# angelvillar96/STLPose

Measured on AMD Instinct MI355X. Metric: images/sec/GPU HRNet-W32 384x288 train step; PCKh@0.5 parity, higher is better.
Workload: dtype f16/bf16; 1 GPU; HRNet-W32 384x288 bs=32/GPU train step (fwd+MSE+bwd+Adam), random-init weights; global_batch=32, parallelism=dp1

## Files before the change

### include/stlpose_hip.h

```cpp
#ifndef STLPOSE_HIP_H
#define STLPOSE_HIP_H
#include <stdint.h>
#ifdef __cplusplus
extern "C" {
#endif

#define STL_F32 0
#define STL_BF16 1
#define STL_F16 2
#define STL_NSHARD 2

#define STL_DT2(grad_dtype, fwd_dtype) ((grad_dtype) | ((fwd_dtype) << 8))

#define STL_SRC_PLAIN 0
#define STL_SRC_BN 1
#define STL_SRC_BNBWD 2
#define STL_SRC_BNADD 3

typedef struct stl_src {
    const void* x;
    const void* y;
    int32_t mode;
    int32_t relu;
    const double* stats;
// ... 127 lines not shown
typedef struct stl_bnrec {
    int64_t stats_off;
    int64_t param_off;
    int64_t buf_off;
    int32_t C;
    float inv_count;
} stl_bnrec;
int stl_bn_running_update(const double* stats, float* buffers, int64_t* num_batches_tracked ,
                          const stl_bnrec* tab, int n, float momentum, int32_t* overflow, void* stream);
int stl_bn_param_grads(const double* rstats, float* grads, const stl_bnrec* tab, int n, void* stream);

int stl_adam_step(float* p, const float* g, float* m, float* v, int64_t n, const float* hyper,
                  int32_t* step, const int32_t* overflow , void* stream);
int stl_sgd_step(float* p, const float* g, float* mom, int64_t n, const float* hyper, int32_t* step,
                 const int32_t* overflow , void* stream);

int stl_affine_crop(const uint8_t* src, const int64_t* src_off, const int32_t* src_hw, const float* minv, const int32_t* flip,
                    float* out, int B, int Ho, int Wo, const float* mean3, const float* std3, void* stream);
int stl_maxpool2x2(int dtype, const void* x, void* out, int B, int H, int W, int C, void* stream);
int stl_l1_partial(int dtype, const void* a, const void* b, int64_t n, double* partial, int nblk,
                   void* stream);
int stl_l2_partial(int dtype, const void* a, const void* b, int64_t n, double* partial, int nblk, void* stream);
int stl_maxpool2x2_backward(int dtype, const void* x, const void* dy, void* dx, int B, int H, int W, int C, int mask, void* stream);
int stl_l2_backward(int dtype, const void* a, const void* b, void* g, int64_t n, const float* scale, int mask, void* stream);
int stl_bilinear_nchw(const float* in, float* out, int B, int C, int H, int W, int Ho, int Wo,
                      void* stream);
int stl_sum_partials(const double* partial, int n, double scale, float* out, int accumulate, void* stream);

int stl_nchw_to_nhwc(int dtype, const float* in, void* out, int B, int C, int H, int W, void* stream);
int stl_nhwc_to_nchw(int dtype, const void* in, float* out, int B, int C, int H, int W, void* stream);
// ... 143 lines not shown
```

### stlpose_amd/capi.py

```python
from __future__ import annotations

import ctypes as C
import os

_HERE = os.path.dirname(os.path.abspath(__file__))
LIB_PATH = os.environ.get("STLPOSE_HIP_LIB") or os.path.join(_HERE, "libstlpose_hip.so")

F32, BF16, F16 = 0, 1, 2


def dt2(grad_dtype: int, fwd_dtype: int) -> int:
    return grad_dtype | ((fwd_dtype if fwd_dtype != grad_dtype else 0) << 8)


POSE_APPROACH = {"all_kpts": 0, "full_body": 1, "upper_body": 2}
POSE_DIM = {"all_kpts": 34, "full_body": 26, "upper_body": 18}
POSE_METHOD = {"euclidean": 0, "cosine": 1, "manhattan": 2, "confidence": 3, "oks": 4, "l2sq": 5, "cos_normalised": 6}
POSE_PEN = {"zero_coord": 0, "none": 1, "mean": 2, "max": 3}
POSE_TOPK_MAX, POSE_RANK_MAX, POSE_RANK_LABELS_MAX, POSE_NSCORES = 1024, 16384, 4, 10
BOX_MAX, RESIZE_SRC_MAX, RESIZE_DST_MAX = 4096, 16384, 2048
DET_NMS_MAX = 65536
GATHER_COPY, GATHER_UP, GATHER_POOL = 0, 1, 2

MIXED = dt2(BF16, F16)
# ... 36 lines not shown


class FuseBwd(C.Structure):
    _fields_ = [("dtype", i32), ("B", i32), ("H", i32), ("W", i32), ("C", i32), ("ngrads", i32), ("relu", i32),
                ("nbn", i32), ("dz", vp * 4), ("z", vp), ("du", vp), ("bn", Src * 4), ("rstats", vp * 4), ("ydtype", i32), ("pad_", i32)]


class UpBwd(C.Structure):
    _fields_ = [("dtype", i32), ("B", i32), ("H", i32), ("W", i32), ("C", i32), ("shift", i32),
                ("du", vp), ("dt", vp), ("bn", Src), ("rstats", vp), ("ydtype", i32), ("pad_", i32)]


class WPrep(C.Structure):
    _fields_ = [("src_off", i64), ("fwd_off", i64), ("bwd_off", i64), ("Co", i32), ("Ci", i32), ("ks", i32),
                ("Cip", i32), ("patch", i32), ("blk0", i32)]


class Slab(C.Structure):
    _fields_ = [("part_off", i64), ("grad_off", i64), ("nsplit", i32), ("Co", i32), ("Ci", i32), ("ks", i32),
                ("Cip", i32), ("patch", i32), ("blk0", i32), ("pad", i32)]


class BNRec(C.Structure):
    _fields_ = [("stats_off", i64), ("param_off", i64), ("buf_off", i64), ("C", i32), ("inv_count", f32)]


class Patch(C.Structure):
    _fields_ = [("dtype", i32), ("B", i32), ("H", i32), ("W", i32), ("stride", i32), ("pad_", i32), ("img", vp), ("out", vp),
                ("mean3", vp), ("std3", vp)]

# ... 65 lines not shown
    "stl_head_forward": [i32, vp, vp, vp, vp, i32, i32, i32, i32, i32, vp],
    "stl_head_backward": [i32, vp, vp, vp, vp, vp, i32, i32, i32, i32, i32, i32, vp],
    "stl_mse_loss": [vp, vp, vp, vp, vp, i32, vp, i32, i32, i32, f32, vp],
    "stl_gaussian_targets": [vp, vp, vp, vp, i32, i32, i32, i32, f32, f32, f32, vp],
    "stl_heatmap_argmax": [vp, vp, vp, vp, i32, i32, i32, vp],
    "stl_flip_merge": [vp, vp, vp, vp, i32, i32, i32, i32, vp],
    "stl_flip_merge_backward": [vp, vp, vp, vp, i32, i32, i32, i32, vp],
    "stl_final_preds": [vp, vp, vp, vp, vp, i32, i32, i32, i32, vp],
    "stl_weight_prep": [i32, vp, vp, vp, i32, i32, vp],
    "stl_reduce_slabs": [vp, vp, vp, i32, i32, vp],
    "stl_reduce_slabs_range": [C.POINTER(ReduceRange), vp],
    "stl_bn_running_update": [vp, vp, vp, vp, i32, f32, vp, vp],
    "stl_bn_param_grads": [vp, vp, vp, i32, vp],
    "stl_adam_step": [vp, vp, vp, vp, i64, vp, vp, vp, vp],
    "stl_sgd_step": [vp, vp, vp, i64, vp, vp, vp, vp],
    "stl_affine_crop": [vp, vp, vp, vp, vp, vp, i32, i32, i32, vp, vp, vp],
    "stl_maxpool2x2": [i32, vp, vp, i32, i32, i32, i32, vp],
    "stl_l1_partial": [i32, vp, vp, i64, vp, i32, vp],
    "stl_l2_partial": [i32, vp, vp, i64, vp, i32, vp],
    "stl_maxpool2x2_backward": [i32, vp, vp, vp, i32, i32, i32, i32, i32, vp],
    "stl_l2_backward": [i32, vp, vp, vp, i64, vp, i32, vp],
    "stl_bilinear_nchw": [vp, vp, i32, i32, i32, i32, i32, i32, vp],
    "stl_sum_partials": [vp, i32, C.c_double, vp, i32, vp],
    "stl_nchw_to_nhwc": [i32, vp, vp, i32, i32, i32, i32, vp],
    "stl_nhwc_to_nchw": [i32, vp, vp, i32, i32, i32, i32, vp],
    "stl_program_create": [C.POINTER(Op), i32, i32, C.POINTER(vp)],
    "stl_program_run": [vp, C.POINTER(vp)],
    "stl_program_run_range": [vp, C.POINTER(vp), i32, i32],
    "stl_program_destroy": [vp],
    "stl_program_wait_op": [vp, i32, vp],
# ... 65 lines not shown
```

### stlpose_amd/csrc/elementwise.hip

```cpp
#include "common.cuh"

namespace {

template <typename T>
__device__ __forceinline__ void load8(const void* base, size_t elem, float* f) {
    if constexpr (sizeof(T) == 2) {
        unpack<T>(ldg16((const char*)base + elem * 2), f);
    } else {
        unpack<float>(ldg16((const char*)base + elem * 4), f);
        unpack<float>(ldg16((const char*)base + elem * 4 + 16), f + 4);
    }
}
template <typename T>
__device__ __forceinline__ void store8(void* base, size_t elem, const float* f) {
    if constexpr (sizeof(T) == 2) {
        stg16((char*)base + elem * 2, pack<T>(f));
    } else {
        stg16((char*)base + elem * 4, pack<float>(f));
        stg16((char*)base + elem * 4 + 16, pack<float>(f + 4));
    }
}

template <int NS>
__device__ __forceinline__ void flush_sets(float (*acc)[8], float* red, int C, int VPC, double* const* dst,
// ... 636 lines not shown
    uint2 u;
    u.x = (uint32_t)__builtin_bit_cast(unsigned short, v[0]) | ((uint32_t)__builtin_bit_cast(unsigned short, v[1]) << 16);
    u.y = (uint32_t)__builtin_bit_cast(unsigned short, v[2]) | ((uint32_t)__builtin_bit_cast(unsigned short, v[3]) << 16);
    *reinterpret_cast<uint2*>(dst) = u;
}
__device__ __forceinline__ void store_vec4(f16* dst, const f16* v) {
    uint2 u;
    u.x = (uint32_t)__builtin_bit_cast(unsigned short, v[0]) | ((uint32_t)__builtin_bit_cast(unsigned short, v[1]) << 16);
    u.y = (uint32_t)__builtin_bit_cast(unsigned short, v[2]) | ((uint32_t)__builtin_bit_cast(unsigned short, v[3]) << 16);
    *reinterpret_cast<uint2*>(dst) = u;
}
__device__ __forceinline__ void store_vec4(float* dst, const float* v) {
    *reinterpret_cast<float4*>(dst) = make_float4(v[0], v[1], v[2], v[3]);
}

template <typename T, typename TF = T>
__global__ __launch_bounds__(256) void weight_prep_kernel(const float* master, T* wk, const stl_wprep* tab, int n, int blk_base) {
    static_assert(sizeof(T) == sizeof(TF), "both layouts live in one buffer of equal-width elements");
    TF* wkf = reinterpret_cast<TF*>(wk);
    const int bx = blockIdx.x + blk_base;
    const int ei = find_entry(&tab[0].blk0, sizeof(stl_wprep) / 4, n, bx);
    const stl_wprep e = tab[ei];
    const int t = e.ks * e.ks;
    const int64_t tot = (int64_t)e.Co * e.Ci * t;
    const int64_t base = (int64_t)(bx - e.blk0) * 1024;
    if (!e.patch && (e.Ci & 3) == 0 && (e.Co & 3) == 0 && t <= 9 && e.Cip == e.Ci && (e.fwd_off & 3) == 0 && (e.bwd_off < 0 || (e.bwd_off & 3) == 0)) {
        __shared__ float st[32 * (32 * 9 + 1)];
        const int pitch = 32 * t + 1;
        const int tci = (e.Ci + 31) >> 5, ntiles = ((e.Co + 31) >> 5) * tci;
        const int nblk = (int)((tot + 1023) / 1024);
        const float* src0 = master + e.src_off;
        for (int tile = bx - e.blk0; tile < ntiles; tile += nblk) {
            const int co0 = (tile / tci) * 32, ci0 = (tile % tci) * 32;
            const int nco = min(32, e.Co - co0), nci = min(32, e.Ci - ci0), seg = nci * t;
            __syncthreads();
            if (((e.src_off & 3) | (int)((uintptr_t)master & 15)) == 0) {
                const int nv = seg >> 2, ntask = nco * nv;
                float4 buf[9];
#pragma unroll
                for (int u = 0; u < 9; ++u) {
                    const int i = threadIdx.x + u * 256;
                    const bool ok = i < ntask;
                    const int r = ok ? i / nv : 0, q = ok ? i - r * nv : 0;
                    buf[u] = *reinterpret_cast<const float4*>(src0 + ((int64_t)(co0 + r) * e.Ci + ci0) * t + 4 * q);
                }
#pragma unroll
                for (int u = 0; u < 9; ++u) {
                    const int i = threadIdx.x + u * 256;
                    if (i < ntask) {
                        const int r = i / nv, q = i - r * nv;
                        float* d = st + r * pitch + 4 * q;
                        d[0] = buf[u].x, d[1] = buf[u].y, d[2] = buf[u].z, d[3] = buf[u].w;
                    }
                }
            } else {
                for (int r = threadIdx.x >> 6; r < nco; r += 4) {
                    const float* row = src0 + ((int64_t)(co0 + r) * e.Ci + ci0) * t;
                    for (int c = threadIdx.x & 63; c < seg; c += 64) st[r * pitch + c] = row[c];
                }
            }
            __syncthreads();
            T v[4];
            TF vf[4];
            const int q4 = nci >> 2;
            for (int i = threadIdx.x; i < nco * t * q4; i += 256) {
                const int row = q4 == 8 ? i >> 3 : i / q4, c4 = (i - row * q4) * 4;
                const int r = t == 9 ? row / 9 : (t == 1 ? row : row / t), tap = row - r * t;
#pragma unroll
                for (int j = 0; j < 4; ++j) vf[j] = (TF)st[r * pitch + (c4 + j) * t + tap];
                store_vec4(wkf + e.fwd_off + ((int64_t)(co0 + r) * t + tap) * e.Ci + ci0 + c4, vf);
            }
            if (e.bwd_off >= 0) {
                const int p4 = nco >> 2;
                for (int i = threadIdx.x; i < nci * t * p4; i += 256) {
                    const int row = p4 == 8 ? i >> 3 : i / p4, r4 = (i - row * p4) * 4;
                    const int c = t == 9 ? row / 9 : (t == 1 ? row : row / t), tapf = row - c * t;
#pragma unroll
                    for (int j = 0; j < 4; ++j) v[j] = (T)st[(r4 + j) * pitch + c * t + (t - 1 - tapf)];
                    store_vec4(wk + e.bwd_off + ((int64_t)(ci0 + c) * t + tapf) * e.Co + co0 + r4, v);
                }
            }
        }
        return;
    }
    for (int r = 0; r < 4; ++r) {
        const int64_t i = base + r * 256 + threadIdx.x;
        if (i >= tot) return;
        const int co = (int)(i / (e.Ci * t)), rem = (int)(i - (int64_t)co * e.Ci * t), ci = rem / t, tap = rem - ci * t;
        const float v = master[e.src_off + i];
        if (e.patch)
            wkf[e.fwd_off + (int64_t)co * e.Cip + tap * e.Ci + ci] = (TF)v;
        else
            wkf[e.fwd_off + ((int64_t)co * t + tap) * e.Cip + ci] = (TF)v;
        if (e.bwd_off >= 0) {
            if (e.patch)
                wk[e.bwd_off + (int64_t)(tap * e.Ci + ci) * e.Co + co] = (T)v;
            else
                wk[e.bwd_off + ((int64_t)ci * t + (t - 1 - tap)) * e.Co + co] = (T)v;
        }
    }
}

__global__ __launch_bounds__(256) void reduce_slabs_kernel(const float* partials, float* grads, const stl_slab* tab, int n, int blk_base) {
    const int bx = blockIdx.x + blk_base;
    const int ei = find_entry(&tab[0].blk0, sizeof(stl_slab) / 4, n, bx);
    const stl_slab e = tab[ei];
    const int t = e.ks * e.ks;
    const int64_t tot = (int64_t)e.Co * e.Ci * t;
    const int tk = e.patch ? 1 : t, cik = e.patch ? e.Cip : e.Ci;
    const int64_t slab = e.pad ? (int64_t)e.pad : (int64_t)e.Co * tk * cik;
    const int64_t base = (int64_t)(bx - e.blk0) * 1024;
    if (!e.patch && (e.Ci & 3) == 0) {
        const int64_t j = base + 4 * threadIdx.x;
        if (j >= tot) return;
        const float* src = partials + e.part_off + j;
// ... 78 lines not shown
        double r1 = 0.0, r2 = 0.0;
        for (int k = 0; k < STL_NSHARD; ++k) {
            r1 += rstats[e.stats_off + (int64_t)k * 2 * e.C + c];
            r2 += rstats[e.stats_off + (int64_t)k * 2 * e.C + e.C + c];
        }
        grads[e.param_off + c] = (float)r2;
        grads[e.param_off + e.C + c] = (float)r1;
    }
}

__global__ void inc_step_kernel(int32_t* step, const int32_t* overflow) {
    const int t = step[0] < 0 ? -step[0] - 1 : step[0];
    step[0] = (overflow && overflow[0] != 0x7fffffff) ? -t - 1 : t + 1;
}

__global__ __launch_bounds__(256) void adam_kernel(float* p, const float* g, float* m, float* v, int64_t n,
                                                   const float* hyper, const int32_t* step) {
    const float lr = hyper[0], b1 = hyper[1], b2 = hyper[2], eps = hyper[3], wd = hyper[4], gs = hyper[7];
    const int t = step[0];
    if (t < 0) return;
    const float bc1 = 1.f - powf(b1, (float)t), bc2 = 1.f - powf(b2, (float)t);
    const float step_size = lr / bc1, isq2 = 1.f / sqrtf(bc2);
    for (int64_t i = (int64_t)blockIdx.x * 256 + threadIdx.x; i < n; i += (int64_t)gridDim.x * 256) {
        float gi = g[i] * gs;
        if (!(fabsf(gi) <= 3.4e38f)) continue;
        const float pi = p[i];
        if (wd != 0.f) gi = fmaf(wd, pi, gi);
        const float mi = b1 * m[i] + (1.f - b1) * gi;
        const float vi = b2 * v[i] + (1.f - b2) * gi * gi;
        m[i] = mi, v[i] = vi;
        p[i] = pi - step_size * mi / (sqrtf(vi) * isq2 + eps);
    }
}

__global__ __launch_bounds__(256) void sgd_kernel(float* p, const float* g, float* mom, int64_t n, const float* hyper,
                                                  const int32_t* step) {
    const float lr = hyper[0], wd = hyper[4], mu = hyper[5], nest = hyper[6], gs = hyper[7];
    if (step[0] < 0) return;
    const bool first = step[0] <= 1;
    for (int64_t i = (int64_t)blockIdx.x * 256 + threadIdx.x; i < n; i += (int64_t)gridDim.x * 256) {
        float gi = g[i] * gs;
        if (!(fabsf(gi) <= 3.4e38f)) continue;
        const float pi = p[i];
        if (wd != 0.f) gi = fmaf(wd, pi, gi);
        if (mu != 0.f) {
            const float b = first ? gi : mu * mom[i] + gi;
            mom[i] = b;
            gi = nest != 0.f ? gi + mu * b : b;
        }
        p[i] = pi - lr * gi;
    }
}


__global__ __launch_bounds__(256) void affine_crop_kernel(const uint8_t* src, const int64_t* src_off, const int32_t* src_hw,
                                                          const float* minv, const int32_t* flip, float* out, int Ho, int Wo,
                                                          const float* mean3, const float* std3) {
    const int b = blockIdx.y;
    const int H = src_hw[2 * b], W = src_hw[2 * b + 1];
    const uint8_t* img = src + src_off[b];
    const float m0 = minv[6 * b], m1 = minv[6 * b + 1], m2 = minv[6 * b + 2];
    const float m3 = minv[6 * b + 3], m4 = minv[6 * b + 4], m5 = minv[6 * b + 5];
    const bool fl = flip && flip[b];
    for (int i = blockIdx.x * 256 + threadIdx.x; i < Ho * Wo; i += gridDim.x * 256) {
        const int y = i / Wo, x = i - y * Wo;
        const float sx = m0 * x + m1 * y + m2, sy = m3 * x + m4 * y + m5;
// ... 507 lines not shown
extern "C" int stl_bn_param_grads(const double* rstats, float* grads, const stl_bnrec* tab, int n, void* stream) {
    if (n == 0) return 0;
    STL_LAUNCH(bn_param_grads_kernel, dim3(n), dim3(256), 0, ST, rstats, grads, tab);
    STL_LAUNCH_CHECK("bn_param_grads");
    return 0;
}

extern "C" int stl_adam_step(float* p, const float* g, float* m, float* v, int64_t n, const float* hyper, int32_t* step, const int32_t* overflow,
                             void* stream) {
    STL_LAUNCH(inc_step_kernel, dim3(1), dim3(1), 0, ST, step, overflow);
    STL_LAUNCH(adam_kernel, dim3(nblocks_for((size_t)n, 256, 4096)), dim3(256), 0, ST, p, g, m, v, n, hyper, step);
    STL_LAUNCH_CHECK("adam_step");
    return 0;
}

extern "C" int stl_sgd_step(float* p, const float* g, float* mom, int64_t n, const float* hyper, int32_t* step, const int32_t* overflow, void* stream) {
    STL_LAUNCH(inc_step_kernel, dim3(1), dim3(1), 0, ST, step, overflow);
    STL_LAUNCH(sgd_kernel, dim3(nblocks_for((size_t)n, 256, 4096)), dim3(256), 0, ST, p, g, mom, n, hyper, step);
    STL_LAUNCH_CHECK("sgd_step");
    return 0;
}

__global__ __launch_bounds__(256) void gaussian_targets_kernel(const float* __restrict__ joints, const float* __restrict__ vis,
                                                               float* __restrict__ target, float* __restrict__ tw, int BJ, int Hh,
                                                               int Wh, double sx, double sy, float sigma) {
    const size_t total = (size_t)BJ * Hh * Wh;
    const float r = sigma * 3.f;
    const float inv2s2 = 1.f / (2.f * sigma * sigma);
    const int c = (int)(2.f * r + 1.f) / 2;
    for (size_t i = (size_t)blockIdx.x * blockDim.x + threadIdx.x; i < total; i += (size_t)gridDim.x * blockDim.x) {
// ... 137 lines not shown
```

### stlpose_amd/engine.py

```python
from __future__ import annotations

import bisect
import ctypes as C
import math
import os
from dataclasses import dataclass, field
from typing import Dict, List, NamedTuple, Optional, Tuple, Union

import torch

from . import capi
from .arch import Arch, Registry, registry, walk

EPS = 1e-5
MOMENTUM = 0.1


def _esz(dtype: int) -> int:
    return 4 if (dtype & 0xff) == capi.F32 else 2


def choose_tile(B: int, Ho: int, Wo: int, stride: int, ks: int, esz: int, bn_cols: int = 64,
                maxpx: int = 128, maxhalo: int = 576) -> Tuple[int, int]:
    vrows = B * (Ho + 1)
# ... 138 lines not shown
        self.nbt_idx: Dict[str, int] = {}
        off, n = 0, 0
        for k, s in reg.buffers:
            if k.endswith("num_batches_tracked"):
                self.nbt_idx[k] = n
                n += 1
            else:
                self.buf_off[k] = off
                off += int(math.prod(s))
        self.nbuf, self.nnbt = off, n
        self.device = device
        self.master = torch.zeros(self.nparam, dtype=torch.float32, device=device)
        self.grads = torch.zeros(self.nparam, dtype=torch.float32, device=device)
        self.bufs = torch.zeros(self.nbuf, dtype=torch.float32, device=device)
        self.nbt = torch.zeros(self.nnbt, dtype=torch.int64, device=device)


class Engine:

    def __init__(self, arch: Arch, store: ParamStore, B: int, H: int, W: int, dtype: int, training: bool,
                 input_grad: bool = False):
        assert H % 32 == 0 and W % 32 == 0, "input H, W must be multiples of 32 (four stride-2 stages + 8x upsample)"
        self.arch, self.store, self.B, self.H, self.W = arch, store, B, H, W
        self.dtype_code = dtype
        self.dtype, self.fdtype = dtype & 0xff, ((dtype >> 8) & 0xff) or (dtype & 0xff)
        self.ydtype = self.fdtype if self.fdtype != self.dtype else 0
        self.training = training
        self.input_grad = input_grad
        self.dev = store.device
        self.esz = _esz(dtype)
# ... 183 lines not shown
        self.fwd_ops.append(Launch("stl_head_forward", hd, 0, [x.ptr], [self.out.data_ptr()]))
        x.consumers += 1
        self.tape.append(HeadNode(x, key, joints))
        return self.out

    def _finalize_weights(self):
        self.wk = torch.zeros(max(self._wk_elems, 1), dtype=self.tdtype, device=self.dev)
        self._resolve("wk", self.wk)
        tab, blk = [], 0
        for c in self.convs:
            tab.append(capi.WPrep(c.master_off, c.fwd_off, c.bwd_off, c.Co, c.Ci, c.ks, c.Cik, int(c.patch), blk))
            blk += math.ceil(c.Co * c.Ci * c.ks * c.ks / 1024)
        self._wprep_blocks = blk
        self._wprep_tab = _to_device((capi.WPrep * len(tab))(*tab), self.dev)
        self._wprep_n = len(self.convs)

    def _active_of(self, key: str) -> int:
        if key.startswith("stage"):
            return int(key[5])
        if key.startswith("transition") and key[10] in "23":
            return int(key[10])
        return 1 if not key.startswith("final") else self.nstreams

    def _new_grad(self, a: Act) -> torch.Tensor:
        return self._act_tensor(a.B, a.H, a.W, a.C)

    def _red(self, bn: BNInfo) -> int:
        return self._red_arena.data_ptr() + 8 * bn.stats_off

    def _build_backward(self):
# ... 334 lines not shown
        self._side = []
        pool = _STREAM_POOL.setdefault(self.dev.index, {})
        with torch.cuda.device(self.dev):
            for i in range(1, n):
                if i not in pool:
                    s_ = torch.cuda.Stream(device=self.dev)
                    pool[i] = (s_, s_.cuda_stream)
                self._side.append(pool[i][0])
                self._stream_arr[i] = pool[i][1]

    def prep_weights(self, stream: int):
        st = self.store
        capi.call("stl_weight_prep", capi.dt2(self.dtype, self.fdtype), st.master.data_ptr(), self.wk.data_ptr(), self._wprep_tab.data_ptr(),
                  self._wprep_n, self._wprep_blocks, stream)

    def forward(self, stream: int, update_running: bool = True):
        self.generation += 1
        self.prep_weights(stream)
        if self.training:
            self.stats.zero_()
        self._run(self._program("fwd"), stream)
        if self.training and update_running:
            st = self.store
            capi.call("stl_bn_running_update", self.stats.data_ptr(), st.bufs.data_ptr(), st.nbt.data_ptr(),
                      self._bn_tab.data_ptr(), len(self.bns), MOMENTUM, self.overflow.data_ptr(), stream)

    NO_OVERFLOW = 2 ** 31 - 1

    def check_forward_range(self):
        i = int(self.overflow.item())
        if i == self.NO_OVERFLOW:
            return
        self.overflow.fill_(self.NO_OVERFLOW)
# ... 38 lines not shown
```

### stlpose_amd/hrnet.py

```python
from __future__ import annotations

import math
import os
from typing import Dict, Optional, Tuple

import torch
import torch.nn as nn

from . import capi, ops
from .arch import ARCHS, Arch, registry
from .engine import Engine, ParamStore


class _Node(nn.Module):

    def forward(self, *a, **k):
        raise RuntimeError("container module; call the top-level network")

    def __getitem__(self, i):
        return self._modules[str(i)]

    def __len__(self):
        return len(self._modules)

# ... 136 lines not shown
                view = st.master[off:off + n].view(shape)
                p = self._tensor(key)
                view.copy_(p.data)
                p.data = view
                p.grad = None
            for key, shape in self._reg.buffers:
                b = self._tensor(key)
                if key.endswith("num_batches_tracked"):
                    view = st.nbt[st.nbt_idx[key]]
                else:
                    off = st.buf_off[key]
                    view = st.bufs[off:off + int(math.prod(shape))].view(shape)
                view.copy_(b)
                mod, leaf = self._leaf[key]
                mod._buffers[leaf] = view
        self._store = st
        self._engines.clear()
        self._anchor = torch.zeros(1, device=device, requires_grad=True)

    def _holder(self):
        ref = self.__dict__.get("_pinned_by")
        return ref() if ref is not None else None

    def __getstate__(self):
        d = dict(self.__dict__)
        for k in ("_pinned_by", "_engines", "_store", "_anchor", "_grad_pub"):
            d.pop(k, None)
        return d

    def __setstate__(self, d):
# ... 57 lines not shown
```

### stlpose_amd/train_step.py

```python
from __future__ import annotations

import os
from typing import List, Optional

import torch

from . import capi
from .dp import FlatAllReduce
from .hrnet import PoseHighResolutionNet

ADAM, SGD = "adam", "sgd"


class TrainStep:
    def __init__(self, model: PoseHighResolutionNet, batch: int, height: int, width: int, optimizer: str = ADAM,
                 lr: float = 1e-3, betas=(0.9, 0.999), eps: float = 1e-8, weight_decay: float = 0.0,
                 momentum: float = 0.9, nesterov: bool = False, process_group=None, bucket_mb: float = 32.0,
                 use_graph: bool = True, device=None, bf16_buckets: Optional[bool] = None):
        self.model = model
        from .hrnet import norm_device
        dev = norm_device(device or "cuda")
        if not model._packed(dev):
            model.to(dev)
            model._pack(dev)
# ... 32 lines not shown
        self.hyper = torch.tensor([lr, betas[0], betas[1], eps, weight_decay, momentum, float(nesterov), gscale],
                                  dtype=torch.float32, device=dev)
        self.step_count = torch.zeros(1, dtype=torch.int32, device=dev)
        J = self.eng.out.shape[1]
        self.target = torch.zeros_like(self.eng.out)
        self.tweight = torch.ones(batch, J, dtype=torch.float32, device=dev)
        self.loss = torch.zeros((), dtype=torch.float32, device=dev)
        self._nblk = 512
        self._partial = torch.zeros(self._nblk, dtype=torch.float64, device=dev)
        if self.eng.nstreams > 1:
            use_graph = False
        self.use_graph = use_graph
        self._g_fb: Optional[torch.cuda.CUDAGraph] = None
        self._g_opt: Optional[torch.cuda.CUDAGraph] = None
        self._loss_scale, self._loss_offset = 1.0, 0.0
        if self.use_graph and process_group is not None:
            self.use_graph = False

    def set_lr(self, lr: float):
        self.hyper[0] = lr

    def set_loss_affine(self, scale: float = 1.0, offset: float = 0.0):
        scale, offset = float(scale), float(offset)
        if self.use_graph and (scale, offset) != (self._loss_scale, self._loss_offset):
            self.use_graph = False
            self._g_fb = self._g_opt = None
        self._loss_scale, self._loss_offset = scale, offset

    def load_batch(self, img: torch.Tensor, target: torch.Tensor, target_weight: torch.Tensor):
        self.eng.img.copy_(img, non_blocking=True)
        self.target.copy_(target, non_blocking=True)
        self.tweight.copy_(target_weight.reshape(self.tweight.shape), non_blocking=True)

    def check_forward_range(self):
        self.eng.check_forward_range()

    def _fwd_bwd(self, update_running: bool = True):
        st = torch.cuda.current_stream().cuda_stream
        e = self.eng
        e.forward(st, update_running=update_running)
        B, J = e.out.shape[:2]
        HW = e.out[0, 0].numel()
        capi.call("stl_mse_loss", e.out.data_ptr(), self.target.data_ptr(), self.tweight.data_ptr(), e.dout.data_ptr(),
                  self._partial.data_ptr(), self._nblk, None, B, J, HW, self._loss_scale, st)
        dp_on = self.dp is not None and (self.world > 1 or self._force_dp) and not self.use_graph and self._dp_rccl
        e.backward(st, on_bucket=self._issue_bucket if dp_on else None)
        self._buckets_issued = dp_on
        capi.call("stl_sum_partials", self._partial.data_ptr(), self._nblk, 0.5 / float(B * J * HW), self.loss.data_ptr(), 0, st)
        if self._loss_scale != 1.0 or self._loss_offset != 0.0:
            self.loss.mul_(self._loss_scale).add_(self._loss_offset)

    def _optim(self):
        st = torch.cuda.current_stream().cuda_stream
        s = self.store
        if self.kind == ADAM:
            capi.call("stl_adam_step", s.master.data_ptr(), s.grads.data_ptr(), self.m.data_ptr(), self.v.data_ptr(),
                      s.nparam, self.hyper.data_ptr(), self.step_count.data_ptr(), self.eng.overflow.data_ptr(), st)
        else:
            capi.call("stl_sgd_step", s.master.data_ptr(), s.grads.data_ptr(), self.m.data_ptr(), s.nparam,
                      self.hyper.data_ptr(), self.step_count.data_ptr(), self.eng.overflow.data_ptr(), st)

    def _issue_bucket(self, i: int):
        if self._comm is None:
            self._comm = torch.cuda.Stream(device=self.dev)
        self.eng.bucket_wait(i, self._comm.cuda_stream)
        with torch.cuda.stream(self._comm):
            self.dp.launch(upto=i + 1, force=self._force_dp)

    def _allreduce(self):
        if self.dp is None or (self.world == 1 and not self._force_dp):
            return
        if not getattr(self, "_buckets_issued", False):
            for i in range(len(self.eng.buckets)):
                self._issue_bucket(i)
        self.dp.wait()
# ... 1 lines not shown
    def _capture(self):
        side = torch.cuda.Stream()
        side.wait_stream(torch.cuda.current_stream())
        with torch.cuda.stream(side):
            self._fwd_bwd(update_running=False)
        torch.cuda.current_stream().wait_stream(side)
        torch.cuda.synchronize()
        self._g_fb = torch.cuda.CUDAGraph()
        with torch.cuda.graph(self._g_fb):
            self._fwd_bwd()
        self._g_opt = torch.cuda.CUDAGraph()
        with torch.cuda.graph(self._g_opt):
            self._optim()

    def step(self) -> torch.Tensor:
        if self.use_graph:
            if self._g_fb is None:
                self._capture()
            self._g_fb.replay()
            self._allreduce()
            self._g_opt.replay()
        else:
            self._fwd_bwd()
            self._allreduce()
            self._optim()
        return self.loss
```

### stlpose_amd/trainer.py

```python
from __future__ import annotations

import json
import os
import time
from typing import Iterable, Optional

import numpy as np
import torch

from .hrnet import PoseHighResolutionNet, norm_device
from .inference import forward_pass
from .loss import PersonMSELoss, perceptual_affine
from .pose_parsing import accuracy
from .train_step import TrainStep

_PREFIX = "module."


def _timestamp() -> str:
    return time.strftime("%Y-%m-%d_%H-%M-%S")


def create_train_logs(exp_path: str) -> dict:
    logs = {"last_modified": _timestamp(), "iterations": 0,
# ... 65 lines not shown
                                                             step_size=int(tr["patience"]))
        else:
            self.scheduler = None
        if self.checkpoint is not None:
            self.load_checkpoint(self.checkpoint, only_model=not self.resume_training)
        self._broadcast_state()

    def _broadcast_state(self):
        if self.world == 1:
            return
        import torch.distributed as dist
        st, ts = self.ts.store, self.ts
        for t in (st.master, st.bufs, st.nbt, ts.m, ts.v, ts.step_count, ts.hyper):
            if t is not None:
                dist.broadcast(t, src=dist.get_global_rank(self.pg, 0), group=self.pg)

    def _mean_over_ranks(self, *vals):
        if self.world == 1:
            return vals
        import torch.distributed as dist
        t = torch.tensor(vals, dtype=torch.float64, device=self.device)
        dist.all_reduce(t, op=dist.ReduceOp.SUM, group=self.pg)
        return tuple((t / self.world).tolist())

    def _common_steps(self, loader) -> Optional[int]:
        if self.world == 1:
            return None
        import torch.distributed as dist
        try:
            n = len(loader)
# ... 154 lines not shown
```

Baseline: 2483 images/sec.

## Fuse optimizer step with low-precision weight prep into one kernel

The Adam/SGD update now runs inside the weight-prep kernel. Each conv weight tile is updated in fp32 and immediately converted into the forward and backward low-precision layouts. Parameters not covered by conv layers are handled by extra gap blocks. The forward pass skips its own weight prep, and a version key triggers a re-prep only when weights change outside the optimizer. This removes one full pass over master weights and one kernel launch per step, at the cost of more complex cache-invalidation logic and weaker occupancy with fewer loads in flight.

```diff
diff --git a/include/stlpose_hip.h b/include/stlpose_hip.h
--- a/include/stlpose_hip.h
+++ b/include/stlpose_hip.h
@@ -165,6 +165,25 @@
                   int32_t* step, const int32_t* overflow , void* stream);
 int stl_sgd_step(float* p, const float* g, float* mom, int64_t n, const float* hyper, int32_t* step,
                  const int32_t* overflow , void* stream);
+
+typedef struct stl_optgap {
+    int64_t off;
+    int32_t n;
+    int32_t blk0;
+} stl_optgap;
+typedef struct stl_optim_prep {
+    int32_t dtype2;
+    int32_t ntab, nblocks;
+    int32_t ngaps, ngapblocks;
+    int32_t pad_;
+    void* wk;
+    const stl_wprep* tab;
+    const stl_optgap* gaps;
+} stl_optim_prep;
+int stl_adam_step_prep(float* p, const float* g, float* m, float* v, const float* hyper, int32_t* step,
+                       const int32_t* overflow , const stl_optim_prep* w, void* stream);
+int stl_sgd_step_prep(float* p, const float* g, float* mom, const float* hyper, int32_t* step,
+                      const int32_t* overflow , const stl_optim_prep* w, void* stream);
 
 int stl_affine_crop(const uint8_t* src, const int64_t* src_off, const int32_t* src_hw, const float* minv, const int32_t* flip,
                     float* out, int B, int Ho, int Wo, const float* mean3, const float* std3, void* stream);
diff --git a/stlpose_amd/capi.py b/stlpose_amd/capi.py
--- a/stlpose_amd/capi.py
+++ b/stlpose_amd/capi.py
@@ -74,6 +74,15 @@
 class WPrep(C.Structure):
     _fields_ = [("src_off", i64), ("fwd_off", i64), ("bwd_off", i64), ("Co", i32), ("Ci", i32), ("ks", i32),
                 ("Cip", i32), ("patch", i32), ("blk0", i32)]
+
+
+class OptGap(C.Structure):
+    _fields_ = [("off", i64), ("n", i32), ("blk0", i32)]
+
+
+class OptimPrep(C.Structure):
+    _fields_ = [("dtype2", i32), ("ntab", i32), ("nblocks", i32), ("ngaps", i32), ("ngapblocks", i32), ("pad_", i32),
+                ("wk", vp), ("tab", vp), ("gaps", vp)]
 
 
 class Slab(C.Structure):
@@ -169,6 +178,8 @@
     "stl_bn_param_grads": [vp, vp, vp, i32, vp],
     "stl_adam_step": [vp, vp, vp, vp, i64, vp, vp, vp, vp],
     "stl_sgd_step": [vp, vp, vp, i64, vp, vp, vp, vp],
+    "stl_adam_step_prep": [vp, vp, vp, vp, vp, vp, vp, C.POINTER(OptimPrep), vp],
+    "stl_sgd_step_prep": [vp, vp, vp, vp, vp, vp, C.POINTER(OptimPrep), vp],
     "stl_affine_crop": [vp, vp, vp, vp, vp, vp, i32, i32, i32, vp, vp, vp],
     "stl_maxpool2x2": [i32, vp, vp, i32, i32, i32, i32, vp],
     "stl_l1_partial": [i32, vp, vp, i64, vp, i32, vp],
diff --git a/stlpose_amd/csrc/elementwise.hip b/stlpose_amd/csrc/elementwise.hip
--- a/stlpose_amd/csrc/elementwise.hip
+++ b/stlpose_amd/csrc/elementwise.hip
@@ -674,11 +674,20 @@
     *reinterpret_cast<float4*>(dst) = make_float4(v[0], v[1], v[2], v[3]);
 }
 
-template <typename T, typename TF = T>
-__global__ __launch_bounds__(256) void weight_prep_kernel(const float* master, T* wk, const stl_wprep* tab, int n, int blk_base) {
+struct src_master {
+    const float* p;
+    typedef float4 pack;
+    static constexpr int inflight = 9;
+    __device__ __forceinline__ bool aligned() const { return ((uintptr_t)p & 15) == 0; }
+    __device__ __forceinline__ pack load4(int64_t i) const { return *reinterpret_cast<const float4*>(p + i); }
+    __device__ __forceinline__ float4 get4(int64_t, const pack& k) const { return k; }
+    __device__ __forceinline__ float get(int64_t i) const { return p[i]; }
+};
+
+template <typename T, typename TF, typename S>
+__device__ __forceinline__ void weight_prep_block(const S& src, T* wk, const stl_wprep* tab, int n, const int bx) {
     static_assert(sizeof(T) == sizeof(TF), "both layouts live in one buffer of equal-width elements");
     TF* wkf = reinterpret_cast<TF*>(wk);
-    const int bx = blockIdx.x + blk_base;
     const int ei = find_entry(&tab[0].blk0, sizeof(stl_wprep) / 4, n, bx);
     const stl_wprep e = tab[ei];
     const int t = e.ks * e.ks;
@@ -689,34 +698,38 @@
         const int pitch = 32 * t + 1;
         const int tci = (e.Ci + 31) >> 5, ntiles = ((e.Co + 31) >> 5) * tci;
         const int nblk = (int)((tot + 1023) / 1024);
-        const float* src0 = master + e.src_off;
         for (int tile = bx - e.blk0; tile < ntiles; tile += nblk) {
             const int co0 = (tile / tci) * 32, ci0 = (tile % tci) * 32;
             const int nco = min(32, e.Co - co0), nci = min(32, e.Ci - ci0), seg = nci * t;
             __syncthreads();
-            if (((e.src_off & 3) | (int)((uintptr_t)master & 15)) == 0) {
+            if ((e.src_off & 3) == 0 && src.aligned()) {
                 const int nv = seg >> 2, ntask = nco * nv;
-                float4 buf[9];
-#pragma unroll
-                for (int u = 0; u < 9; ++u) {
-                    const int i = threadIdx.x + u * 256;
-                    const bool ok = i < ntask;
-                    const int r = ok ? i / nv : 0, q = ok ? i - r * nv : 0;
-                    buf[u] = *reinterpret_cast<const float4*>(src0 + ((int64_t)(co0 + r) * e.Ci + ci0) * t + 4 * q);
-                }
-#pragma unroll
-                for (int u = 0; u < 9; ++u) {
-                    const int i = threadIdx.x + u * 256;
-                    if (i < ntask) {
-                        const int r = i / nv, q = i - r * nv;
-                        float* d = st + r * pitch + 4 * q;
-                        d[0] = buf[u].x, d[1] = buf[u].y, d[2] = buf[u].z, d[3] = buf[u].w;
+                typename S::pack buf[S::inflight];
+#pragma unroll
+                for (int u0 = 0; u0 < 9; u0 += S::inflight) {
+#pragma unroll
+                    for (int u = 0; u < S::inflight; ++u) {
+                        const int i = threadIdx.x + (u0 + u) * 256;
+                        if (i < ntask) {
+                            const int r = i / nv, q = i - r * nv;
+                            buf[u] = src.load4(e.src_off + ((int64_t)(co0 + r) * e.Ci + ci0) * t + 4 * q);
+                        }
+                    }
+#pragma unroll
+                    for (int u = 0; u < S::inflight; ++u) {
+                        const int i = threadIdx.x + (u0 + u) * 256;
+                        if (i < ntask) {
+                            const int r = i / nv, q = i - r * nv;
+                            const float4 w = src.get4(e.src_off + ((int64_t)(co0 + r) * e.Ci + ci0) * t + 4 * q, buf[u]);
+                            float* d = st + r * pitch + 4 * q;
+                            d[0] = w.x, d[1] = w.y, d[2] = w.z, d[3] = w.w;
+                        }
                     }
                 }
             } else {
                 for (int r = threadIdx.x >> 6; r < nco; r += 4) {
-                    const float* row = src0 + ((int64_t)(co0 + r) * e.Ci + ci0) * t;
-                    for (int c = threadIdx.x & 63; c < seg; c += 64) st[r * pitch + c] = row[c];
+                    const int64_t row = e.src_off + ((int64_t)(co0 + r) * e.Ci + ci0) * t;
+                    for (int c = threadIdx.x & 63; c < seg; c += 64) st[r * pitch + c] = src.get(row + c);
                 }
             }
             __syncthreads();
@@ -747,7 +760,7 @@
         const int64_t i = base + r * 256 + threadIdx.x;
         if (i >= tot) return;
         const int co = (int)(i / (e.Ci * t)), rem = (int)(i - (int64_t)co * e.Ci * t), ci = rem / t, tap = rem - ci * t;
-        const float v = master[e.src_off + i];
+        const float v = src.get(e.src_off + i);
         if (e.patch)
             wkf[e.fwd_off + (int64_t)co * e.Cip + tap * e.Ci + ci] = (TF)v;
         else
@@ -759,6 +772,11 @@
                 wk[e.bwd_off + ((int64_t)ci * t + (t - 1 - tap)) * e.Co + co] = (T)v;
         }
     }
+}
+
+template <typename T, typename TF = T>
+__global__ __launch_bounds__(256) void weight_prep_kernel(const float* master, T* wk, const stl_wprep* tab, int n, int blk_base) {
+    weight_prep_block<T, TF>(src_master{master}, wk, tab, n, (int)blockIdx.x + blk_base);
 }
 
 __global__ __launch_bounds__(256) void reduce_slabs_kernel(const float* partials, float* grads, const stl_slab* tab, int n, int blk_base) {
@@ -867,42 +885,159 @@
     step[0] = (overflow && overflow[0] != 0x7fffffff) ? -t - 1 : t + 1;
 }
 
+struct adam_math {
+    float b1, b2, eps, wd, gs, step_size, isq2;
+    __device__ __forceinline__ void init(const float* hyper, int t) {
+        const float lr = hyper[0];
+        b1 = hyper[1], b2 = hyper[2], eps = hyper[3], wd = hyper[4], gs = hyper[7];
+        const float bc1 = 1.f - powf(b1, (float)t), bc2 = 1.f - powf(b2, (float)t);
+        step_size = lr / bc1, isq2 = 1.f / sqrtf(bc2);
+    }
+    __device__ __forceinline__ bool upd(float& pi, float gi, float& mi, float& vi) const {
+        gi = gi * gs;
+        if (!(fabsf(gi) <= 3.4e38f)) return false;
+        if (wd != 0.f) gi = fmaf(wd, pi, gi);
+        mi = b1 * mi + (1.f - b1) * gi;
+        vi = b2 * vi + (1.f - b2) * gi * gi;
+        pi = pi - step_size * mi / (sqrtf(vi) * isq2 + eps);
+        return true;
+    }
+};
+
+struct sgd_math {
+    float lr, wd, mu, nest, gs;
+    bool first;
+    __device__ __forceinline__ void init(const float* hyper, int t) {
+        lr = hyper[0], wd = hyper[4], mu = hyper[5], nest = hyper[6], gs = hyper[7];
+        first = t <= 1;
+    }
+    __device__ __forceinline__ bool upd(float& pi, float gi, float& bi) const {
+        gi = gi * gs;
+        if (!(fabsf(gi) <= 3.4e38f)) return false;
+        if (wd != 0.f) gi = fmaf(wd, pi, gi);
+        if (mu != 0.f) {
+            bi = first ? gi : mu * bi + gi;
+            gi = nest != 0.f ? gi + mu * bi : bi;
+        }
+        pi = pi - lr * gi;
+        return true;
+    }
+};
+
 __global__ __launch_bounds__(256) void adam_kernel(float* p, const float* g, float* m, float* v, int64_t n,
                                                    const float* hyper, const int32_t* step) {
-    const float lr = hyper[0], b1 = hyper[1], b2 = hyper[2], eps = hyper[3], wd = hyper[4], gs = hyper[7];
     const int t = step[0];
     if (t < 0) return;
-    const float bc1 = 1.f - powf(b1, (float)t), bc2 = 1.f - powf(b2, (float)t);
-    const float step_size = lr / bc1, isq2 = 1.f / sqrtf(bc2);
+    adam_math a;
+    a.init(hyper, t);
     for (int64_t i = (int64_t)blockIdx.x * 256 + threadIdx.x; i < n; i += (int64_t)gridDim.x * 256) {
-        float gi = g[i] * gs;
-        if (!(fabsf(gi) <= 3.4e38f)) continue;
-        const float pi = p[i];
-        if (wd != 0.f) gi = fmaf(wd, pi, gi);
-        const float mi = b1 * m[i] + (1.f - b1) * gi;
-        const float vi = b2 * v[i] + (1.f - b2) * gi * gi;
+        float pi = p[i], mi = m[i], vi = v[i];
+        if (!a.upd(pi, g[i], mi, vi)) continue;
         m[i] = mi, v[i] = vi;
-        p[i] = pi - step_size * mi / (sqrtf(vi) * isq2 + eps);
+        p[i] = pi;
     }
 }
 
 __global__ __launch_bounds__(256) void sgd_kernel(float* p, const float* g, float* mom, int64_t n, const float* hyper,
                                                   const int32_t* step) {
-    const float lr = hyper[0], wd = hyper[4], mu = hyper[5], nest = hyper[6], gs = hyper[7];
     if (step[0] < 0) return;
-    const bool first = step[0] <= 1;
+    sgd_math a;
+    a.init(hyper, step[0]);
     for (int64_t i = (int64_t)blockIdx.x * 256 + threadIdx.x; i < n; i += (int64_t)gridDim.x * 256) {
-        float gi = g[i] * gs;
-        if (!(fabsf(gi) <= 3.4e38f)) continue;
-        const float pi = p[i];
-        if (wd != 0.f) gi = fmaf(wd, pi, gi);
-        if (mu != 0.f) {
-            const float b = first ? gi : mu * mom[i] + gi;
-            mom[i] = b;
-            gi = nest != 0.f ? gi + mu * b : b;
-        }
-        p[i] = pi - lr * gi;
-    }
+        float pi = p[i], bi = a.mu != 0.f ? mom[i] : 0.f;
+        if (!a.upd(pi, g[i], bi)) continue;
+        if (a.mu != 0.f) mom[i] = bi;
+        p[i] = pi;
+    }
+}
+
+struct src_adam {
+    float* p; const float* g; float* m; float* v;
+    adam_math a;
+    struct pack { float4 p, g, m, v; };
+    static constexpr int inflight = 3;
+    __device__ __forceinline__ bool aligned() const { return (((uintptr_t)p | (uintptr_t)g | (uintptr_t)m | (uintptr_t)v) & 15) == 0; }
+    __device__ __forceinline__ pack load4(int64_t i) const {
+        pack k;
+        k.p = *reinterpret_cast<const float4*>(p + i), k.g = *reinterpret_cast<const float4*>(g + i);
+        k.m = *reinterpret_cast<const float4*>(m + i), k.v = *reinterpret_cast<const float4*>(v + i);
+        return k;
+    }
+    __device__ __forceinline__ float4 get4(int64_t i, pack k) const {
+        const bool any = a.upd(k.p.x, k.g.x, k.m.x, k.v.x) | a.upd(k.p.y, k.g.y, k.m.y, k.v.y) |
+                         a.upd(k.p.z, k.g.z, k.m.z, k.v.z) | a.upd(k.p.w, k.g.w, k.m.w, k.v.w);
+        if (any) {
+            *reinterpret_cast<float4*>(m + i) = k.m, *reinterpret_cast<float4*>(v + i) = k.v;
+            *reinterpret_cast<float4*>(p + i) = k.p;
+        }
+        return k.p;
+    }
+    __device__ __forceinline__ float get(int64_t i) const {
+        float pi = p[i], mi = m[i], vi = v[i];
+        if (a.upd(pi, g[i], mi, vi)) m[i] = mi, v[i] = vi, p[i] = pi;
+        return pi;
+    }
+};
+
+struct src_sgd {
+    float* p; const float* g; float* mom;
+    sgd_math a;
+    struct pack { float4 p, g, b; };
+    static constexpr int inflight = 3;
+    __device__ __forceinline__ bool aligned() const { return (((uintptr_t)p | (uintptr_t)g | (uintptr_t)mom) & 15) == 0; }
+    __device__ __forceinline__ pack load4(int64_t i) const {
+        pack k;
+        k.p = *reinterpret_cast<const float4*>(p + i), k.g = *reinterpret_cast<const float4*>(g + i);
+        k.b = a.mu != 0.f ? *reinterpret_cast<const float4*>(mom + i) : make_float4(0.f, 0.f, 0.f, 0.f);
+        return k;
+    }
+    __device__ __forceinline__ float4 get4(int64_t i, pack k) const {
+        const bool any = a.upd(k.p.x, k.g.x, k.b.x) | a.upd(k.p.y, k.g.y, k.b.y) | a.upd(k.p.z, k.g.z, k.b.z) | a.upd(k.p.w, k.g.w, k.b.w);
+        if (any) {
+            if (a.mu != 0.f) *reinterpret_cast<float4*>(mom + i) = k.b;
+            *reinterpret_cast<float4*>(p + i) = k.p;
+        }
+        return k.p;
+    }
+    __device__ __forceinline__ float get(int64_t i) const {
+        float pi = p[i], bi = a.mu != 0.f ? mom[i] : 0.f;
+        if (a.upd(pi, g[i], bi)) {
+            if (a.mu != 0.f) mom[i] = bi;
+            p[i] = pi;
+        }
+        return pi;
+    }
+};
+
+template <typename T, typename TF, typename S>
+__device__ __forceinline__ void optim_prep_body(S& src, const float* hyper, const int32_t* step, T* wk, const stl_wprep* tab,
+                                                int n, int nblocks, const stl_optgap* gaps, int ngaps) {
+    const int t = step[0];
+    if (t < 0) return;
+    src.a.init(hyper, t);
+    if ((int)blockIdx.x < nblocks) {
+        weight_prep_block<T, TF>(src, wk, tab, n, (int)blockIdx.x);
+        return;
+    }
+    const int bx = (int)blockIdx.x - nblocks;
+    const int ei = find_entry(&gaps[0].blk0, sizeof(stl_optgap) / 4, ngaps, bx);
+    const int64_t off = gaps[ei].off;
+    const int cnt = gaps[ei].n, base = (bx - gaps[ei].blk0) * 1024;
+    for (int r = 0; r < 4; ++r) {
+        const int j = base + r * 256 + (int)threadIdx.x;
+        if (j < cnt) src.get(off + j);
+    }
+}
+
+template <typename T, typename TF>
+__global__ __launch_bounds__(256) void adam_kernel_prep(src_adam src, const float* hyper, const int32_t* step, T* wk, const stl_wprep* tab,
+                                                        int n, int nblocks, const stl_optgap* gaps, int ngaps) {
+    optim_prep_body<T, TF>(src, hyper, step, wk, tab, n, nblocks, gaps, ngaps);
+}
+template <typename T, typename TF>
+__global__ __launch_bounds__(256) void sgd_kernel_prep(src_sgd src, const float* hyper, const int32_t* step, T* wk, const stl_wprep* tab,
+                                                       int n, int nblocks, const stl_optgap* gaps, int ngaps) {
+    optim_prep_body<T, TF>(src, hyper, step, wk, tab, n, nblocks, gaps, ngaps);
 }
 
 
@@ -1440,6 +1575,54 @@
     return 0;
 }
 
+template <typename S>
+static int optim_prep_launch(const S& src, const float* hyper, int32_t* step, const int32_t* overflow, const stl_optim_prep* w, void* stream,
+                             const char* what) {
+    STL_CHECK(w && w->wk && w->tab && w->ntab > 0 && w->nblocks > 0 && w->ngaps >= 0 && w->ngapblocks >= 0 && (w->ngaps == 0 || w->gaps),
+              "%s: bad weight table", what);
+    const int dtype = w->dtype2 & 0xff, fdtype = (w->dtype2 >> 8) & 0xff;
+    STL_CHECK(fdtype == 0 || fdtype == dtype || (dtype == STL_BF16 && fdtype == STL_F16), "%s: forward type %d does not go with %d", what, fdtype, dtype);
+    const dim3 grid(w->nblocks + (w->ngaps ? w->ngapblocks : 0));
+    STL_LAUNCH(inc_step_kernel, dim3(1), dim3(1), 0, ST, step, overflow);
+#define OPTIM_PREP_LAUNCH(T, TF)                                                                                                   \
+    do {                                                                                                                           \
+        if constexpr (std::is_same<S, src_adam>::value)                                                                            \
+            STL_LAUNCH((adam_kernel_prep<T, TF>), grid, dim3(256), 0, ST, src, hyper, step, (T*)w->wk, w->tab, w->ntab, w->nblocks, w->gaps, w->ngaps); \
+        else                                                                                                                       \
+            STL_LAUNCH((sgd_kernel_prep<T, TF>), grid, dim3(256), 0, ST, src, hyper, step, (T*)w->wk, w->tab, w->ntab, w->nblocks, w->gaps, w->ngaps);  \
+    } while (0)
+    if (dtype == STL_BF16 && fdtype == STL_F16)
+        OPTIM_PREP_LAUNCH(__bf16, f16);
+    else if (dtype == STL_F16)
+        OPTIM_PREP_LAUNCH(f16, f16);
+    else if (dtype == STL_BF16)
+        OPTIM_PREP_LAUNCH(__bf16, __bf16);
+    else
+        OPTIM_PREP_LAUNCH(float, float);
+#undef OPTIM_PREP_LAUNCH
+    return 0;
+}
+
+extern "C" int stl_adam_step_prep(float* p, const float* g, float* m, float* v, const float* hyper, int32_t* step, const int32_t* overflow,
+                                  const stl_optim_prep* w, void* stream) {
+    STL_CHECK(p && g && m && v && hyper && step, "adam_step_prep: null pointer");
+    src_adam src;
+    src.p = p, src.g = g, src.m = m, src.v = v;
+    if (optim_prep_launch(src, hyper, step, overflow, w, stream, "adam_step_prep")) return 1;
+    STL_LAUNCH_CHECK("adam_step_prep");
+    return 0;
+}
+
+extern "C" int stl_sgd_step_prep(float* p, const float* g, float* mom, const float* hyper, int32_t* step, const int32_t* overflow,
+                                 const stl_optim_prep* w, void* stream) {
+    STL_CHECK(p && g && mom && hyper && step, "sgd_step_prep: null pointer");
+    src_sgd src;
+    src.p = p, src.g = g, src.mom = mom;
+    if (optim_prep_launch(src, hyper, step, overflow, w, stream, "sgd_step_prep")) return 1;
+    STL_LAUNCH_CHECK("sgd_step_prep");
+    return 0;
+}
+
 extern "C" int stl_sgd_step(float* p, const float* g, float* mom, int64_t n, const float* hyper, int32_t* step, const int32_t* overflow, void* stream) {
     STL_LAUNCH(inc_step_kernel, dim3(1), dim3(1), 0, ST, step, overflow);
     STL_LAUNCH(sgd_kernel, dim3(nblocks_for((size_t)n, 256, 4096)), dim3(256), 0, ST, p, g, mom, n, hyper, step);
diff --git a/stlpose_amd/engine.py b/stlpose_amd/engine.py
--- a/stlpose_amd/engine.py
+++ b/stlpose_amd/engine.py
@@ -176,6 +176,14 @@
         self.grads = torch.zeros(self.nparam, dtype=torch.float32, device=device)
         self.bufs = torch.zeros(self.nbuf, dtype=torch.float32, device=device)
         self.nbt = torch.zeros(self.nnbt, dtype=torch.int64, device=device)
+        self.epoch = 0
+        self.watch: List[torch.Tensor] = []
+
+    def touch(self):
+        self.epoch += 1
+
+    def weights_key(self) -> Tuple[int, int]:
+        return self.epoch, self.master._version + sum(p._version for p in self.watch)
 
 
 class Engine:
@@ -389,6 +397,20 @@
         self._wprep_blocks = blk
         self._wprep_tab = _to_device((capi.WPrep * len(tab))(*tab), self.dev)
         self._wprep_n = len(self.convs)
+        gaps, gblk, at = [], 0, 0
+        for c in sorted(self.convs, key=lambda c: c.master_off):
+            assert c.master_off >= at, "two conv layers share a weight: the fused optimiser would step it twice"
+            if c.master_off > at:
+                gaps.append(capi.OptGap(at, c.master_off - at, gblk))
+                gblk += math.ceil((c.master_off - at) / 1024)
+            at = c.master_off + c.Co * c.Ci * c.ks * c.ks
+        if at < self.store.nparam:
+            gaps.append(capi.OptGap(at, self.store.nparam - at, gblk))
+            gblk += math.ceil((self.store.nparam - at) / 1024)
+        self._gap_tab = _to_device((capi.OptGap * len(gaps))(*gaps), self.dev) if gaps else None
+        op = self.optim_prep = capi.OptimPrep()
+        op.dtype2, op.ntab, op.nblocks, op.ngaps, op.ngapblocks = capi.dt2(self.dtype, self.fdtype), self._wprep_n, blk, len(gaps), gblk
+        op.wk, op.tab, op.gaps = self.wk.data_ptr(), self._wprep_tab.data_ptr(), self._gap_tab.data_ptr() if gaps else None
 
     def _active_of(self, key: str) -> int:
         if key.startswith("stage"):
@@ -753,9 +775,10 @@
         capi.call("stl_weight_prep", capi.dt2(self.dtype, self.fdtype), st.master.data_ptr(), self.wk.data_ptr(), self._wprep_tab.data_ptr(),
                   self._wprep_n, self._wprep_blocks, stream)
 
-    def forward(self, stream: int, update_running: bool = True):
+    def forward(self, stream: int, update_running: bool = True, prep: bool = True):
         self.generation += 1
-        self.prep_weights(stream)
+        if prep:
+            self.prep_weights(stream)
         if self.training:
             self.stats.zero_()
         self._run(self._program("fwd"), stream)
diff --git a/stlpose_amd/hrnet.py b/stlpose_amd/hrnet.py
--- a/stlpose_amd/hrnet.py
+++ b/stlpose_amd/hrnet.py
@@ -174,6 +174,7 @@
                 view.copy_(b)
                 mod, leaf = self._leaf[key]
                 mod._buffers[leaf] = view
+        st.watch = [self._tensor(key) for key, shape in self._reg.params if len(shape) == 4]
         self._store = st
         self._engines.clear()
         self._anchor = torch.zeros(1, device=device, requires_grad=True)
diff --git a/stlpose_amd/train_step.py b/stlpose_amd/train_step.py
--- a/stlpose_amd/train_step.py
+++ b/stlpose_amd/train_step.py
@@ -1,5 +1,6 @@
 from __future__ import annotations
 
+import ctypes
 import os
 from typing import List, Optional
 
@@ -70,6 +71,7 @@
         self._g_fb: Optional[torch.cuda.CUDAGraph] = None
         self._g_opt: Optional[torch.cuda.CUDAGraph] = None
         self._loss_scale, self._loss_offset = 1.0, 0.0
+        self._wk_key = None
         if self.use_graph and process_group is not None:
             self.use_graph = False
 
@@ -91,10 +93,16 @@
     def check_forward_range(self):
         self.eng.check_forward_range()
 
+    def _prep_weights(self):
+        key = self.store.weights_key()
+        if key != self._wk_key:
+            self.eng.prep_weights(torch.cuda.current_stream().cuda_stream)
+            self._wk_key = key
+
     def _fwd_bwd(self, update_running: bool = True):
         st = torch.cuda.current_stream().cuda_stream
         e = self.eng
-        e.forward(st, update_running=update_running)
+        e.forward(st, update_running=update_running, prep=False)
         B, J = e.out.shape[:2]
         HW = e.out[0, 0].numel()
         capi.call("stl_mse_loss", e.out.data_ptr(), self.target.data_ptr(), self.tweight.data_ptr(), e.dout.data_ptr(),
@@ -109,12 +117,17 @@
     def _optim(self):
         st = torch.cuda.current_stream().cuda_stream
         s = self.store
+        wp = ctypes.byref(self.eng.optim_prep)
         if self.kind == ADAM:
-            capi.call("stl_adam_step", s.master.data_ptr(), s.grads.data_ptr(), self.m.data_ptr(), self.v.data_ptr(),
-                      s.nparam, self.hyper.data_ptr(), self.step_count.data_ptr(), self.eng.overflow.data_ptr(), st)
+            capi.call("stl_adam_step_prep", s.master.data_ptr(), s.grads.data_ptr(), self.m.data_ptr(), self.v.data_ptr(),
+                      self.hyper.data_ptr(), self.step_count.data_ptr(), self.eng.overflow.data_ptr(), wp, st)
         else:
-            capi.call("stl_sgd_step", s.master.data_ptr(), s.grads.data_ptr(), self.m.data_ptr(), s.nparam,
-                      self.hyper.data_ptr(), self.step_count.data_ptr(), self.eng.overflow.data_ptr(), st)
+            capi.call("stl_sgd_step_prep", s.master.data_ptr(), s.grads.data_ptr(), self.m.data_ptr(),
+                      self.hyper.data_ptr(), self.step_count.data_ptr(), self.eng.overflow.data_ptr(), wp, st)
+
+    def _optim_done(self):
+        self.store.touch()
+        self._wk_key = self.store.weights_key()
 
     def _issue_bucket(self, i: int):
         if self._comm is None:
@@ -146,6 +159,7 @@
             self._optim()
 
     def step(self) -> torch.Tensor:
+        self._prep_weights()
         if self.use_graph:
             if self._g_fb is None:
                 self._capture()
@@ -156,4 +170,5 @@
             self._fwd_bwd()
             self._allreduce()
             self._optim()
+        self._optim_done()
         return self.loss
diff --git a/stlpose_amd/trainer.py b/stlpose_amd/trainer.py
--- a/stlpose_amd/trainer.py
+++ b/stlpose_amd/trainer.py
@@ -103,6 +103,7 @@
         for t in (st.master, st.bufs, st.nbt, ts.m, ts.v, ts.step_count, ts.hyper):
             if t is not None:
                 dist.broadcast(t, src=dist.get_global_rank(self.pg, 0), group=self.pg)
+        st.touch()
 
     def _mean_over_ranks(self, *vals):
         if self.world == 1:
```

Result: no change. 2482 images/sec (-0.0%).
